# Teachable-AI-Lab/RAG-Cobweb

Measured on AMD Instinct MI355X. Metric: queries/sec + recall@10 vs FAISS-flat, 1M×768 corpus, 1/2/4/8 MI355X, higher is better.
Workload: dtype f32

## Files before the change

### rag-cobweb_amd/csrc/cwq_mfma.hip

```cpp
#include <hip/hip_runtime.h>
#include <math.h>
#include <stdint.h>

#include <algorithm>
#include <type_traits>

#include "cwq_internal.h"

namespace cwq {

typedef __bf16 bf16x8 __attribute__((ext_vector_type(8)));
typedef float f32x16 __attribute__((ext_vector_type(16)));
typedef float f32x4 __attribute__((ext_vector_type(4)));
typedef int i32x4 __attribute__((ext_vector_type(4)));
typedef float f32x2 __attribute__((ext_vector_type(2)));
typedef __attribute__((address_space(3))) void lds_void;
typedef __attribute__((address_space(1))) void glb_void;

#define CWQ_INF __builtin_inff()

__device__ __forceinline__ float up(double v) { return (float)(v * (1.0 + 0x1p-20)); }

__global__ void rows_prep_kernel(const float* __restrict__ mean, int D, const int64_t* __restrict__ nodes, int64_t n,
                                 const float* __restrict__ c, int DP, int DPB, int64_t ld, float* Mf, __bf16* Mb,
// ... 246 lines not shown
    float sc;
    i8_split_wave([&](int d) { return (valid && d < a.D) ? xq[d] - cq[d] : 0.f; }, a.DPB,
                  reinterpret_cast<int8_t*>(a.Xq) + r * a.DPB, sv, shi, slo, sc);
    if (lane == 0) a.qinfo8[r] = make_float4((float)sv, up(sqrt(shi)), up(sqrt(slo)), sc);
  }
  if (!valid) return;
  if (tid < 5) a.qcnt[(size_t)tid * a.nq + r] = 0;
  if (r == 0 && tid == 5) a.qcnt[(size_t)5 * a.nq] = 0;
  if (a.NI == 0) return;
  float* part = s_sb + 2 * DQ;
  for (int t = tid; t < a.NI * NV16; t += 256) {
    const int n = t / NV16, v = t - n * NV16;
    float pp;
#pragma unroll
    for (int j = 0; j < 16; ++j) {
      const int d = v * 16 + j;
      const float x = xq[d];
      const float tt = fmaf(x, a.A[(size_t)d * a.ld + n], -a.B[(size_t)d * a.ld + n]);
      pp = (j == 0) ? tt * tt : fmaf(tt, tt, pp);
    }
    part[t] = pp;
  }
  __syncthreads();
  float* Pl = part + a.NI * NV16;
  for (int lv = 0; lv < a.nlev; ++lv) {
    for (int i = a.lv0[lv] + tid; i < a.lv0[lv + 1]; i += 256) {
      const float acc = sum_in_order(part + i * NV16, NV16);
      const float lp = -0.5f * (a.logdet_int[i] + acc);
      const int p = a.par_int[i];
      const float P = p >= 0 ? fmaf(a.w_int[i], lp, Pl[p]) : a.w_int[i] * lp;
      Pl[i] = P;
      a.P[(size_t)r * a.ldP + i] = P;
    }
    __syncthreads();
  }
}

hipError_t launch_sb_prep(const SbPrepArgs& a, hipStream_t s) {
  const size_t lds = ((size_t)2 * std::max(a.DP, a.DPB) + (size_t)a.NI * (a.DP / 16) + a.NI) * 4;
  if (a.nq <= 0 || a.nq_pad < a.nq16 || a.nq16 < a.nq || a.DP % 16 || a.NI > kSbMaxNI || a.nlev > kSbMaxNI ||
      lds > 65536)
    return hipErrorInvalidValue;
  hipLaunchKernelGGL(sb_prep_kernel, dim3((unsigned)a.nq_pad), dim3(256), lds, s, a);
  return hipGetLastError();
}

__device__ __forceinline__ void prefix_step(float pl, float ph, float w, float& lo, float& hi) {
  const float a = w >= 0.f ? lo : hi, b = w >= 0.f ? hi : lo;
  const float m = 0x1p-21f * (fmaxf(fabsf(pl), fabsf(ph)) + fabsf(w) * fmaxf(fabsf(lo), fabsf(hi)));
  lo = fmaf(w, a, pl) - m;
  hi = fmaf(w, b, ph) + m;
}

__global__ void int_prep_kernel(const float* __restrict__ mean, const VarSrc var, int D,
                                const int64_t* __restrict__ nodes, int64_t n, const float* __restrict__ c,
                                const float* __restrict__ logdet, const int* __restrict__ par_int,
                                const float* __restrict__ w_int, int DP, int DPB2, int64_t ld, __bf16* Mb2, RowF* rf,
                                float* Ar, float* Br, float gamma) {
  const int lane = threadIdx.x & 63;
  const int64_t r = blockIdx.x * (int64_t)kWavesPerWG + (threadIdx.x >> 6);
  if (r >= ld) return;
  double shi = 0.0, slo = 0.0, cn = 0.0, mn = 0.0;
  float wmax = 0.f;
  for (int k = lane; k < DPB2; k += kWave) {
    const int d = k < DP ? k : k - DP;
    const bool ok = r < n && k < 2 * DP && d < D;
    float v = 0.f;
    if (ok) {
      const int64_t o = nodes[r] * (int64_t)D + d;
      const float A = 1.0f / sqrtf(var.at(nodes[r], d, D));
      const float w = A * A;
      const float mu = mean[o];
      const float mc = mu - c[d];
      if (k < DP) {
        v = -0.5f * w;
        const double am = fabs((double)mu) + fabs((double)c[d]);
        cn += (double)mc * (double)mc * (double)w;
        mn += (double)w * am * am;
        wmax = fmaxf(wmax, w);
        Ar[r * DP + d] = A;
        Br[r * DP + d] = mu * A;
      } else {
        v = mc * w;
      }
    } else if (r < n && k < DP) {
      Ar[r * DP + k] = 0.f;
      Br[r * DP + k] = 0.f;
    }
    const __bf16 h = (__bf16)v;
    const float hf = (float)h;
    const float lo = v - hf;
    if (Mb2) Mb2[r * DPB2 + k] = h;
    shi += (double)hf * (double)hf;
    slo += (double)lo * (double)lo;
  }
  for (int off = 32; off > 0; off >>= 1) {
    shi += __shfl_xor(shi, off, 64);
    slo += __shfl_xor(slo, off, 64);
    cn += __shfl_xor(cn, off, 64);
    mn += __shfl_xor(mn, off, 64);
    wmax = fmaxf(wmax, __shfl_xor(wmax, off, 64));
  }
  if (lane == 0) {
    RowF f;
    if (r < n) {
      const double bh = sqrt(shi) * (1.0 + 0x1p-20), bl = sqrt(slo) * (1.0 + 0x1p-20);
      f.R0 = up(mn);
      f.beta = up(bl + (double)gamma * bh);
      f.delta = up(bh + bl);
      f.rn2 = (float)cn;
      f.hs = wmax;
      f.hl = logdet[r];
      f.invL = w_int[r];
      f.par = par_int[r];
    } else {
      f = RowF{0.f, 0.f, 0.f, 0.f, 0.f, 0.f, 0.f, -2};
    }
    if (rf) rf[r] = f;
  }
}

hipError_t launch_int_prep(const float* mean, const VarSrc& var, int D, const int64_t* nodes, int64_t n,
                           const float* c, const float* logdet, const int* par_int, const float* w_int, int DP, int DPB2,
                           int64_t ld, void* Mb2, RowF* rf, float* Ar, float* Br, float gamma, hipStream_t s) {
  if (ld <= 0) return hipSuccess;
  hipLaunchKernelGGL(int_prep_kernel, dim3((unsigned)((ld + 3) / 4)), dim3(256), 0, s, mean, var, D, nodes, n, c,
                     logdet, par_int, w_int, DP, DPB2, ld, (__bf16*)Mb2, rf, Ar, Br, gamma);
  return hipGetLastError();
}

__global__ void int_path_prep_kernel(const float* __restrict__ mean, const VarSrc var, int D,
                                     const int64_t* __restrict__ nodes, const int* __restrict__ rows, int64_t n,
                                     const float* __restrict__ c, const float* __restrict__ logdet,
                                     const int* __restrict__ par_int, const float* __restrict__ w_int, int DP, int DPB2,
                                     int64_t ld, __bf16* Mb2, RowF* rf, float gamma) {
  const int lane = threadIdx.x & 63;
  const int64_t r = blockIdx.x * (int64_t)kWavesPerWG + (threadIdx.x >> 6);
  if (r >= ld) return;
  const int i = r < n ? rows[r] : -1;
  double K0 = 0.0, Z0 = 0.0, Z3 = 0.0;
  int depth = 0;
  for (int a = i; a >= 0 && par_int[a] >= 0; a = par_int[a]) {
    ++depth;
    const int64_t nd = nodes[a];
    double cn = 0.0, mn = 0.0;
    float wmax = 0.f;
    for (int d = lane; d < D; d += kWave) {
      const float A = 1.0f / sqrtf(var.at(nd, d, D));
      const float w = A * A;
      const float mu = mean[nd * (int64_t)D + d];
      const float mc = mu - c[d];
      const double am = fabs((double)mu) + fabs((double)c[d]);
      cn += (double)mc * (double)mc * (double)w;
      mn += (double)w * am * am;
      wmax = fmaxf(wmax, w);
    }
    for (int off = 32; off > 0; off >>= 1) {
      cn += __shfl_xor(cn, off, 64);
      mn += __shfl_xor(mn, off, 64);
      wmax = fmaxf(wmax, __shfl_xor(wmax, off, 64));
    }
    const double wa = (double)w_int[a], ld_a = (double)logdet[a];
    K0 += -0.5 * wa * (ld_a + cn);
    Z0 += fabs(wa) * (mn + fabs(ld_a) + cn);
    Z3 += fabs(wa) * (double)wmax;
  }
  double shi = 0.0, slo = 0.0;
  for (int k = lane; k < DPB2; k += kWave) {
    const int d = k < DP ? k : k - DP;
    double acc = 0.0;
    if (k < 2 * DP && d < D)
      for (int a = i; a >= 0 && par_int[a] >= 0; a = par_int[a]) {
        const int64_t nd = nodes[a];
        const float A = 1.0f / sqrtf(var.at(nd, d, D));
        const float w = A * A;
        const float v = k < DP ? -0.5f * w : (mean[nd * (int64_t)D + d] - c[d]) * w;
        acc += (double)w_int[a] * (double)v;
      }
    const float v = (float)acc;
    const __bf16 h = (__bf16)v;
    const float hf = (float)h;
    const float lo = v - hf;
    Mb2[r * DPB2 + k] = h;
    shi += (double)hf * (double)hf;
    slo += (double)lo * (double)lo;
  }
  for (int off = 32; off > 0; off >>= 1) {
    shi += __shfl_xor(shi, off, 64);
    slo += __shfl_xor(slo, off, 64);
  }
  if (lane == 0) {
    RowF f = RowF{0.f, 0.f, 0.f, 0.f, 0.f, 0.f, 0.f, -2};
    if (i >= 0) {
      f.par = par_int[i];
      if (f.par >= 0) {
        const double bh = sqrt(shi) * (1.0 + 0x1p-20), bl = sqrt(slo) * (1.0 + 0x1p-20);
        const double cz = 1.02 * (0x1p-12 + depth * 0x1p-24);
        f.beta = up(bl + (double)gamma * bh);
        f.delta = up(bh + bl);
        f.rn2 = (float)K0;
        f.hs = up(cz * Z3);
        f.R0 = up(cz * Z0 + 0x1p-23 * fabs(K0));
        f.hl = up(depth * 0x1p-24 + 0x1p-22);
      }
    }
    rf[r] = f;
  }
}

hipError_t launch_int_path_prep(const float* mean, const VarSrc& var, int D, const int64_t* nodes, const int* rows,
                                int64_t n, const float* c, const float* logdet, const int* par_int,
                                const float* w_int, int DP, int DPB2, int64_t ld, void* Mb2, RowF* rf, float gamma,
                                hipStream_t s) {
  if (ld <= 0) return hipSuccess;
  hipLaunchKernelGGL(int_path_prep_kernel, dim3((unsigned)((ld + 3) / 4)), dim3(256), 0, s, mean, var, D, nodes, rows,
                     n, c, logdet, par_int, w_int, DP, DPB2, ld, (__bf16*)Mb2, rf, gamma);
  return hipGetLastError();
}

__global__ void query_prep2_kernel(const float* __restrict__ q, int64_t nq, int D, const float* __restrict__ c,
                                   int DP, int DPB2, int64_t nq_pad, __bf16* Xb2, float4* qinfo) {
  const int lane = threadIdx.x & 63;
  const int64_t r = blockIdx.x * (int64_t)kWavesPerWG + (threadIdx.x >> 6);
  if (r >= nq_pad) return;
  double shi = 0.0, slo = 0.0, sx = 0.0;
  for (int k = lane; k < DPB2; k += kWave) {
    const int d = k < DP ? k : k - DP;
    float v = 0.f;
    if (r < nq && k < 2 * DP && d < D) {
      const float x = q[r * D + d];
      const float xc = x - c[d];
      v = k < DP ? xc * xc : xc;
      if (k < DP) sx += (double)x * (double)x + (double)xc * (double)xc;
    }
    const __bf16 h = (__bf16)v;
    const float hf = (float)h;
    const float lo = v - hf;
    Xb2[r * DPB2 + k] = h;
    shi += (double)hf * (double)hf;
    slo += (double)lo * (double)lo;
  }
  for (int off = 32; off > 0; off >>= 1) {
    shi += __shfl_xor(shi, off, 64);
    slo += __shfl_xor(slo, off, 64);
    sx += __shfl_xor(sx, off, 64);
  }
  if (lane == 0) qinfo[r] = make_float4(up(sx), up(sqrt(shi)), up(sqrt(slo)), 0.f);
}

hipError_t launch_query_prep2(const float* q, int64_t nq, int D, const float* c, int DP, int DPB2, int64_t nq_pad,
                              void* Xb2, float4* qinfo, hipStream_t s) {
  hipLaunchKernelGGL(query_prep2_kernel, dim3((unsigned)((nq_pad + 3) / 4)), dim3(256), 0, s, q, nq, D, c, DP, DPB2,
                     nq_pad, (__bf16*)Xb2, qinfo);
  return hipGetLastError();
}

__global__ void prefix_bounds_kernel(float* Plo, float* Phi, int64_t ldP, int nq, int i0, int i1,
                                     const int* __restrict__ par_int, const float* __restrict__ w_int,
                                     const float* __restrict__ logdet_int, const float* __restrict__ Sroot) {
  const int n = i1 - i0;
  const int64_t total = (int64_t)n * nq;
  for (int64_t t = blockIdx.x * (int64_t)blockDim.x + threadIdx.x; t < total; t += (int64_t)gridDim.x * blockDim.x) {
    const int q = (int)(t / n);
    const int i = i0 + (int)(t % n);
    const size_t o = (size_t)q * ldP + i;
    const int p = par_int[i];
    const float w = w_int[i];
    if (p < 0) {
      const float lp = -0.5f * (logdet_int[i] + Sroot[q]);
      const float P = w * lp;
      Plo[o] = P;
      Phi[o] = P;
      continue;
    }
    const size_t op = (size_t)q * ldP + p;
    float lo = Plo[o], hi = Phi[o];
    prefix_step(Plo[op], Phi[op], w, lo, hi);
    Plo[o] = lo;
    Phi[o] = hi;
  }
}

hipError_t launch_prefix_bounds(float* Plo, float* Phi, int64_t ldP, int nq, int i0, int i1, const int* par_int,
                                const float* w_int, const float* logdet_int, const float* Sroot, hipStream_t s) {
  const int64_t total = (int64_t)(i1 - i0) * nq;
  if (total <= 0) return hipSuccess;
  dim3 grid((unsigned)std::min<int64_t>((total + 255) / 256, 8192));
  hipLaunchKernelGGL(prefix_bounds_kernel, grid, dim3(256), 0, s, Plo, Phi, ldP, nq, i0, i1, par_int, w_int,
                     logdet_int, Sroot);
  return hipGetLastError();
}

constexpr int FT = kFgTile;
constexpr int FK = 32;
constexpr int FNBUF = 4;
constexpr int FSTAGE = 2 * FT * FK * 2;
constexpr int OFF_QV = FNBUF * FSTAGE;
constexpr int OFF_QI = OFF_QV + FT * 4;
constexpr int OFF_PI = OFF_QI + FT * 16;
constexpr int OFF_PL = OFF_PI + FT * 4;
constexpr int OFF_REC = OFF_PL + FT * 4;
constexpr int OFF_CNT = OFF_REC + kFgCap * 16;
constexpr int FLDS = OFF_CNT + 128;


__device__ __forceinline__ void int_bounds(float dot, float4 qi, const RowF& f, float gamma, float& lo, float& hi) {
  (void)gamma;
  const float S0 = fmaf(-2.f, dot, f.rn2);
  const float E = 2.f * (fmaf(qi.y, f.beta, qi.z * f.delta) + 0x1p-23f * fabsf(dot)) + 0x1p-20f * fabsf(f.rn2) +
                  0x1p-12f * fmaf(f.hs, qi.x, f.R0);
  const float Eu = E * (1.f + 0x1p-20f);
  const float Shi = (S0 + Eu) * (1.f + 0x1p-22f);
  const float Slo = fmaxf(0.f, (S0 - Eu) * (1.f - 0x1p-22f));
  const float m = 0x1p-20f * (fabsf(f.hl) + Shi);
  hi = -0.5f * (f.hl + Slo) + m;
  lo = -0.5f * (f.hl + Shi) - m;
}

__device__ __forceinline__ void fg_decode(const FgArgs& a, int xcd, int i, int& qt, int& rt) {
  const int qg = xcd % a.qgroups, rg = xcd / a.qgroups;
  const int nqt_g = (a.n_qt + a.qgroups - 1) / a.qgroups;
  const int nrt_g = (a.n_rt + a.rgroups - 1) / a.rgroups;
  const int q_lo = qg * nqt_g, r_lo = rg * nrt_g;
  const int nq_l = max(1, min(nqt_g, a.n_qt - q_lo));
  const int nr_l = max(1, min(nrt_g, a.n_rt - r_lo));
  if (a.order == 1) {
    qt = q_lo + i / nr_l;
    rt = a.rt_off + r_lo + i % nr_l;
  } else {
    qt = q_lo + i % nq_l;
    rt = a.rt_off + r_lo + i / nq_l;
  }
}

__device__ __forceinline__ int fg_count(const FgArgs& a, int xcd) {
  const int qg = xcd % a.qgroups, rg = xcd / a.qgroups;
  const int nqt_g = (a.n_qt + a.qgroups - 1) / a.qgroups;
  const int nrt_g = (a.n_rt + a.rgroups - 1) / a.rgroups;
  const int nq_l = max(0, min(nqt_g, a.n_qt - qg * nqt_g));
  const int nr_l = max(0, min(nrt_g, a.n_rt - rg * nrt_g));
  return nq_l * nr_l;
}

#ifndef FG_STAMP
#define FG_STAMP 0
#endif
#ifndef FG_LEAN
#define FG_LEAN 1
#endif
#define FG_CSLOT (FG_LEAN && !RAW && MODE == 0 && (tile_no & 1) ? 9 : 0)
__device__ __forceinline__ int fg_swz(int r) { return (4 - ((r >> 2) & 3)) & 3; }

template <int ES = 2>
__device__ __forceinline__ void fg_stage(const __bf16* __restrict__ Xb, const __bf16* __restrict__ Mb, int DPB, int q0,
                                         int r0, int k0, char* sb, int wave, const uint32_t* loff, int ipart = -1) {
  const char* gA = reinterpret_cast<const char*>(Xb) + ((size_t)q0 * DPB + k0) * ES;
  const char* gB = reinterpret_cast<const char*>(Mb) + ((size_t)r0 * DPB + k0) * ES;
#pragma unroll
  for (int i = 0; i < 2; ++i) {
    if (ipart >= 0 && i != ipart) continue;
    __builtin_amdgcn_global_load_lds((glb_void*)(gA + loff[i]), (lds_void*)(sb + (wave * 32 + i * 16) * 64), 16, 0, 0);
    __builtin_amdgcn_global_load_lds((glb_void*)(gB + loff[i]), (lds_void*)(sb + FT * 64 + (wave * 32 + i * 16) * 64), 16,
                                     0, 0);
  }
}

__device__ __forceinline__ TileF fg_tile_const(const TileF* p, int i) {
  static_assert(sizeof(TileF) == 32, "TileF is 8 dwords");
  typedef const __attribute__((address_space(4))) int* cip;
  const cip src = (cip)(uintptr_t)(p + i);
  TileF t;
  int* d = reinterpret_cast<int*>(&t);
#pragma unroll
  for (int k = 0; k < 8; ++k) d[k] = src[k];
  return t;
}

template <bool I8 = false>
__device__ __forceinline__ bool fg_raw_bounds(const FgArgs& a, int q, int row, float d, float ex, float& u,
                                              float& lo) {
  const RowF f = (I8 ? a.rf8 : a.rf)[row];
  if (f.par < -1) return false;
  const TileF tf = a.tf[row / kFgTile];
  float Pq = 0.f, Pql = 0.f;
  if (tf.par >= 0) {
    if (a.pb.dot) {
      pathb_bounds(a.pb, q, tf.par, Pql, Pq);
    } else {
      Pq = (a.Phi ? a.Phi : a.P)[pidx(a.ldP, a.pT, q, tf.par)];
      Pql = a.P[pidx(a.ldP, a.pT, q, tf.par)];
    }
  }
  const float pi = __fmul_rn(Pq, tf.invL), pl = __fmul_rn(Pql, tf.invL);
  fg_bounds2(d, ex, (I8 ? a.qinfo8 : a.qinfo)[q], f, pi, pl, a.eps_n, a.slack, u, lo);
  return u >= a.T[(size_t)q * a.ldT];
}

template <int MODE, bool ALLUNI, bool RAW = false, bool I8 = false>
__global__ __launch_bounds__(512) void fgemm_kernel(const __bf16* __restrict__ Xb, const __bf16* __restrict__ Mb,
                                                    const FgArgs a) {
  static_assert(!I8 || RAW, "int8 operands: raw-record launches only");
  typedef typename std::conditional<I8, i32x4, bf16x8>::type frag_t;
  typedef typename std::conditional<I8, i32x4, f32x4>::type acc_t;
  constexpr int ES = I8 ? 1 : 2;
  constexpr int SK = 64 / ES;
  __shared__ __attribute__((aligned(16))) char smem[FLDS + (I8 ? 2 * FT * 8 : 0)];
  const int tid = threadIdx.x;
  const int lane = tid & 63;
  const int wave = __builtin_amdgcn_readfirstlane(tid >> 6);
  const int wq = wave & 1, wr = wave >> 1;
  const int xcd = blockIdx.x & 7;
  const int lw = blockIdx.x >> 3;
  const int nw_x = ((int)gridDim.x - xcd + 7) >> 3;
  const int ntl = fg_count(a, xcd);
  const bool dyn = a.order == 2;
  if (!dyn && lw >= ntl) return;
  const int nk = a.DPB / SK;
  float* s_qv = reinterpret_cast<float*>(smem + OFF_QV);
  float4* s_qi = reinterpret_cast<float4*>(smem + OFF_QI);
  float* s_pi = reinterpret_cast<float*>(smem + OFF_PI);
  float* s_pl = reinterpret_cast<float*>(smem + OFF_PL);
  const float* Pu = a.Phi ? a.Phi : a.P;
  auto pboth = [&](int64_t q, int p, float& lo, float& hi) {
    if (a.pb.dot) {
      pathb_bounds(a.pb, q, p, lo, hi);
    } else {
      lo = a.P[pidx(a.ldP, a.pT, q, p)];
      hi = Pu[pidx(a.ldP, a.pT, q, p)];
    }
  };
  int4* s_rec = reinterpret_cast<int4*>(smem + OFF_REC);
  int* s_cnt = reinterpret_cast<int*>(smem + OFF_CNT);
  static_assert(!RAW || (MODE == 0 && ALLUNI), "raw records: all-uniform filter launches only");
  static_assert(kFgCap == 512, "the record flush copies one record per thread");
  auto flush_records = [&](int cnt) {
    const int n = min(cnt, kFgCap);
    if (tid == 0) {
      int chunk = s_cnt[1], fill = s_cnt[2];
      int n1 = chunk >= 0 ? min(n, kFgChunk - fill) : 0;
      int base1 = chunk * kFgChunk + fill, base2 = 0, nw = n;
      fill += n1;
      if (n > n1) {
        if (chunk >= 0) a.chunk_fill[chunk] = fill;
        const int c2 = atomicAdd(a.gctr, 1);
        if ((int64_t)(c2 + 1) * kFgChunk > a.rec_cap) {
          chunk = -1;
          fill = 0;
          nw = n1;
        } else {
          chunk = c2;
          fill = n - n1;
          base2 = c2 * kFgChunk;
        }
      }
      s_cnt[1] = chunk;
      s_cnt[2] = fill;
      s_cnt[3] = base1;
      s_cnt[4] = n1;
      s_cnt[5] = nw;
      s_cnt[6] = base2;
    }
    __syncthreads();
    const int nw = s_cnt[5], n1 = s_cnt[4];
    if (tid < nw) a.rec[tid < n1 ? s_cnt[3] + tid : s_cnt[6] + (tid - n1)] = s_rec[tid];
    else if (tid < n) a.qover[s_rec[tid].x] = 1;
    if (tid == 0) s_cnt[0] = 0;
  };
  uint32_t loff[2];
#pragma unroll
  for (int i = 0; i < 2; ++i) {
    const int row = wave * 32 + i * 16 + (lane >> 2);
    loff[i] = (uint32_t)((row * a.DPB + (((lane & 3) ^ fg_swz(row)) * (16 / ES))) * ES);
  }
  const int r16 = lane & 15, c16 = lane >> 4;
  const int foff16 = r16 * 64 + ((c16 ^ fg_swz(r16)) << 4);

  int i = lw;
  if (dyn) {
    if (tid == 0) s_cnt[8] = atomicAdd(&a.tctr[xcd], 1);
    __syncthreads();
    i = __builtin_amdgcn_readfirstlane(s_cnt[8]);
    if (i >= ntl) return;
  }
  int next_i = dyn ? ntl : i + nw_x;
  int ic_i = i, ic_k = 0, ic_qt, ic_rt, issued = 0, gs = 0;
  fg_decode(a, xcd, ic_i, ic_qt, ic_rt);
  auto issue_next = [&]() {
    if (ic_i == -2) {
      ic_i = next_i;
      if (ic_i < ntl) fg_decode(a, xcd, ic_i, ic_qt, ic_rt);
    }
    if (ic_i >= ntl) return;
    if (!(a.dbg & 1)) fg_stage<ES>(Xb, Mb, a.DPB, ic_qt * FT, ic_rt * FT, ic_k * SK, smem + (issued & (FNBUF - 1)) * FSTAGE, wave, loff);
    ++issued;
    if (++ic_k == nk) {
      ic_k = 0;
      ic_i = -2;
    }
  };
  issue_next();
  issue_next();
  if (!I8 || nk >= 3) issue_next();
  int qt, rt;
  int tile_no = 0;
  (void)tile_no;
  fg_decode(a, xcd, i, qt, rt);
  if (tid == 0) {
    s_cnt[0] = 0;
    s_cnt[9] = 0;
    s_cnt[1] = -1;
    s_cnt[2] = 0;
  }
  if (RAW && lane == 0) s_cnt[16 + wave] = 0;
  acc_t acc[8][4];
#if FG_STAMP
  unsigned long long* tsp = (a.stamp && blockIdx.x < 64 && tid == 0) ? a.stamp + 16384 + (size_t)blockIdx.x * 128 : nullptr;
#define FG_TS(k)                                                                  \
  do {                                                                            \
    if (tsp && tile_no < 16) tsp[tile_no * 8 + (k)] = __builtin_amdgcn_s_memtime(); \
  } while (0)
#else
#define FG_TS(k) \
  do {           \
  } while (0)
#endif
  for (;;) {
    FG_TS(0);
    const int q0 = qt * FT, r0 = rt * FT;
    TileF tf;
    if (MODE == 0) tf = fg_tile_const(I8 ? a.tf8 : a.tf, rt);
    else tf.uniform = 0;
    const bool uni = ALLUNI || tf.uniform != 0;
    const bool multi = !ALLUNI && tf.uniform == 2;
    int claimv = 0;
    if (dyn && tid == 0) {
      int z;
      asm volatile("v_mov_b32 %0, 0" : "=v"(z));
      claimv = atomicAdd(a.tctr + xcd + z, 1);
    }
    const int qs = q0 + tid;
    float4 qi = make_float4(0.f, 0.f, 0.f, 0.f);
    float Tq = CWQ_INF, Pq = 0.f, Pql = 0.f;
    float2 rw8 = make_float2(-CWQ_INF, 0.f);
    (void)rw8;
    if (tid < FT) {
      qi = (I8 ? a.qinfo8 : a.qinfo)[qs];
      if (qs < a.nq && MODE == 0) Tq = a.T[(size_t)qs * a.ldT];
      if (uni && tf.par >= 0 && qs < a.nq) {
        if (a.pb.dot) {
          pathb_bounds(a.pb, qs, tf.par, Pql, Pq);
        } else {
          Pq = Pu[pidx(a.ldP, a.pT, qs, tf.par)];
          Pql = a.P[pidx(a.ldP, a.pT, qs, tf.par)];
        }
      }
      if (I8 && r0 + tid < a.nrows) rw8 = make_float2(a.rf[r0 + tid].R0, a.rf8[r0 + tid].R0);
    }
    float R0[4], SR[4];
    (void)SR;
#pragma unroll
    for (int jb = 0; jb < 4; ++jb) {
      if (I8) break;
      const int r = r0 + wr * 64 + jb * 16 + r16;
      R0[jb] = (uni && r < a.nrows) ? a.rf[r].R0 : RAW ? -CWQ_INF : 0.f;
    }
    float* const s_qvt = RAW && (tile_no & 1) ? reinterpret_cast<float*>(smem + OFF_QI) : s_qv;
    if (tid < FT) {
      const float T = Tq;
      if constexpr (I8) {
        (tile_no & 1 ? s_pl : s_pi)[tid] = qi.w;
        reinterpret_cast<float2*>(smem + FLDS)[(tile_no & 1) * FT + tid] = rw8;
      }
      qi.w = T;
      if (!RAW) s_qi[tid] = qi;
      auto qv_of = [&](float pi) {
        const float tpg = (T - pi) / tf.g;
        float v = qi.x * (0.5f - 0.5f * a.eps_n) - 1.5f * a.slack * qi.x + tpg - a.slack * fabsf(pi) / tf.g -
                  qi.y * tf.beta_max - qi.z * tf.delta_max;
        v -= 4.f * a.gamma * (fabsf(v) + qi.x + fabsf(tpg) + fabsf(pi) / tf.g);
        return v == v ? v : CWQ_INF;
      };
      float pi = 0.f, qv = CWQ_INF;
      if (uni) {
        pi = Pq * tf.invL;
        if (qs < a.nq && T > -CWQ_INF) {
          qv = qv_of(pi);
          if (multi) {
            const float2 pm = a.pmm[(size_t)rt * a.ldq + qs];
            const float A = qi.x * (0.5f - 0.5f * a.eps_n) - 1.5f * a.slack * qi.x - qi.y * tf.beta_max -
                            qi.z * tf.delta_max;
            const float M = fmaxf(fabsf(pm.x), fabsf(pm.y));
            const float v1L = A + (T - pm.y) / tf.g - a.slack * M / tf.g;
            const float v1U = A + (T - pm.x) / tf.g;
            const float tpm = fmaxf(fabsf(T - pm.x), fabsf(T - pm.y)) / tf.g;
            const float v = v1L - 4.f * a.gamma * (fmaxf(fabsf(v1L), fabsf(v1U)) + qi.x + tpm + M / tf.g);
            qv = v == v ? fminf(qv, v) : CWQ_INF;
          }
        }
      }
      if (!RAW) {
        s_pi[tid] = pi;
        s_pl[tid] = uni ? Pql * tf.invL : 0.f;
      }
      if (MODE == 2) s_pl[tid] = qs < a.nq ? a.root_w * (-0.5f * (a.root_ld + a.Sroot[qs])) : 0.f;
      s_qvt[tid] = qv;
    }
    if (dyn && tid == 0) s_cnt[8] = claimv;
    __syncthreads();
    FG_TS(1);
    if (dyn) next_i = __builtin_amdgcn_readfirstlane(s_cnt[8]);
    if (FG_LEAN && !RAW && MODE == 0 && tid == 0 && tile_no > 0) s_cnt[(tile_no & 1) ? 0 : 9] = 0;
    if (RAW) {
      const int cnt = s_cnt[0];
      if (cnt >= kFgCap / 2) flush_records(cnt);
    }
#pragma unroll
    for (int ib = 0; ib < 8; ++ib) {
      if constexpr (I8) {
#pragma unroll
        for (int jb = 0; jb < 4; ++jb) acc[ib][jb] = acc_t{0, 0, 0, 0};
      } else {
        const float4 qv4 = uni ? *reinterpret_cast<const float4*>(s_qvt + wq * 128 + ib * 16 + 4 * c16)
                               : make_float4(0.f, 0.f, 0.f, 0.f);
#pragma unroll
        for (int jb = 0; jb < 4; ++jb) {
          acc[ib][jb][0] = R0[jb] - qv4.x;
          acc[ib][jb][1] = R0[jb] - qv4.y;
          acc[ib][jb][2] = R0[jb] - qv4.z;
          acc[ib][jb][3] = R0[jb] - qv4.w;
        }
      }
    }
    frag_t xa1[8], xb0[4];
    const int grp = wave >> 2;
    auto sbar = [&]() {
      __builtin_amdgcn_sched_barrier(0);
      __builtin_amdgcn_s_barrier();
      __builtin_amdgcn_sched_barrier(0);
    };
    if (grp) sbar();
#if FG_STAMP
    const bool stp = a.stamp && blockIdx.x < 16 && (wave & 3) == 0 && lane == 0 && tile_no >= 4 && tile_no < 6;
    unsigned long long* sp =
        stp ? a.stamp + ((((size_t)blockIdx.x * 2 + (tile_no - 4)) * 2 + (wave >> 2)) * 32) * 6 : nullptr;
#define FG_ST(k)                                                               \
  do {                                                                         \
    if (stp && t < 32) sp[t * 6 + (k)] = __builtin_amdgcn_s_memtime();         \
  } while (0)
#else
#define FG_ST(k) \
  do {           \
  } while (0)
#endif
    for (int t = 0; t < nk; ++t) {
      FG_ST(0);
      const char* sb = smem + (gs & (FNBUF - 1)) * FSTAGE;
      issue_next();
      if (!(a.dbg & 128)) {
        const char* sA = sb + wq * 128 * 64 + foff16;
        const char* sB = sb + FT * 64 + wr * 64 * 64 + foff16;
#pragma unroll
        for (int ib = 0; ib < 8; ++ib) xa1[ib] = *reinterpret_cast<const frag_t*>(sA + ib * 1024);
#pragma unroll
        for (int jb = 0; jb < 4; ++jb) xb0[jb] = *reinterpret_cast<const frag_t*>(sB + jb * 1024);
      }
      ++gs;
      const int n_out = issued - gs - 1;
      if (a.dbg & 256) asm volatile("s_waitcnt lgkmcnt(0)" ::: "memory");
      else if (n_out >= 2) asm volatile("s_waitcnt vmcnt(8) lgkmcnt(0)" ::: "memory");
      else if (n_out == 1) asm volatile("s_waitcnt vmcnt(4) lgkmcnt(0)" ::: "memory");
      else asm volatile("s_waitcnt vmcnt(0) lgkmcnt(0)" ::: "memory");
      FG_ST(1);
      sbar();
      FG_ST(2);
#pragma unroll
      for (int ib = 0; ib < 8; ++ib)
#pragma unroll
        for (int jb = 0; jb < 4; ++jb) {
          if constexpr (I8) acc[ib][jb] = __builtin_amdgcn_mfma_i32_16x16x64_i8(xa1[ib], xb0[jb], acc[ib][jb], 0, 0, 0);
          else acc[ib][jb] = __builtin_amdgcn_mfma_f32_16x16x32_bf16(xa1[ib], xb0[jb], acc[ib][jb], 0, 0, 0);
        }
      FG_ST(3);
      if (t + 1 < nk || grp == 0) sbar();
      FG_ST(4);
    }
#undef FG_ST
    FG_TS(2);
    float* wsc = reinterpret_cast<float*>(smem + ((gs - 1) & (FNBUF - 1)) * FSTAGE) + wave * 1024;
    bool anyb[4][2];
    if (a.dbg & 2) goto flush;
    if (MODE == 2 && a.pT) {
      int par[4], rid[4];
#pragma unroll
      for (int jb = 0; jb < 4; ++jb) {
        const int r = r0 + wr * 64 + jb * 16 + r16;
        par[jb] = r < a.nrows ? a.rf[r].par : -2;
        rid[jb] = r < a.nrows ? a.row_id[r] : -1;
      }
#pragma unroll
      for (int ib = 0; ib < 8; ++ib) {
        const int ql = wq * 128 + ib * 16 + 4 * c16;
        const int q = q0 + ql;
        if (q >= a.ldlb) continue;
#pragma unroll
        for (int jb = 0; jb < 4; ++jb) {
          if (par[jb] < -1 || rid[jb] < 0) continue;
          const size_t o = (size_t)rid[jb] * a.ldlb + q;
          const float4 v = par[jb] < 0 ? *reinterpret_cast<const float4*>(s_pl + ql)
                                       : make_float4(acc[ib][jb][0], acc[ib][jb][1], acc[ib][jb][2], acc[ib][jb][3]);
          *reinterpret_cast<float4*>(a.lb + o) = v;
        }
      }
      goto flush;
    }
    if (MODE == 2) {
      const int rl = r0 + wr * 64 + lane;
      const RowF f = rl < a.nrows ? a.rf[rl] : RowF{0.f, 0.f, 0.f, 0.f, 0.f, 0.f, 0.f, -2};
      const int rid = a.row_id ? (rl < a.nrows ? a.row_id[rl] : -1) : rl;
#pragma unroll
      for (int ib = 0; ib < 8; ++ib) {
#pragma unroll
        for (int jb = 0; jb < 4; ++jb)
#pragma unroll
          for (int j = 0; j < 4; ++j) wsc[(4 * c16 + j) * 64 + jb * 16 + r16] = acc[ib][jb][j];
        __builtin_amdgcn_fence(__ATOMIC_RELEASE, "wavefront");
        __builtin_amdgcn_wave_barrier();
        __builtin_amdgcn_fence(__ATOMIC_ACQUIRE, "wavefront");
#pragma unroll 4
        for (int e = 0; e < 16; ++e) {
          const int ql = wq * 128 + ib * 16 + e;
          const int q = q0 + ql;
          if (f.par >= -1 && q < a.nq) {
            const float d0 = wsc[e * 64 + lane];
            float lo, hi;
            if (f.par < 0) {
              lo = hi = s_pl[ql];
            } else if (a.path_sum) {
              path_bounds(d0, s_qi[ql], f, s_pl[ql], lo, hi);
            } else {
              int_bounds(d0, s_qi[ql], f, a.gamma, lo, hi);
              if (f.par == 0) prefix_step(s_pl[ql], s_pl[ql], f.invL, lo, hi);
            }
            a.lb[(size_t)q * a.ldlb + rid] = lo;
            a.lb_hi[(size_t)q * a.ldlb + rid] = hi;
          }
        }
        __builtin_amdgcn_wave_barrier();
      }
      goto flush;
    }
    if (MODE == 1 && a.lbg == 4 && !a.pb.dot) {
      int rrow[4];
      float pa[4], pb[4];
#pragma unroll
      for (int jb = 0; jb < 4; ++jb) {
        const int r = r0 + wr * 64 + jb * 16 + r16;
        const int rr = a.rowmap ? a.rowmap[r] : (r < a.nrows ? r : -1);
        const RowF f = rr >= 0 ? a.rf[rr] : RowF{-CWQ_INF, 0.f, 0.f, 0.f, 0.f, 0.f, 0.f, -2};
        rrow[jb] = f.par >= -1 ? rr : -1;
        pa[jb] = fmaf(f.hs, f.rn2, f.hl);
        pb[jb] = -2.f * f.hs;
      }
      const int g = (r0 + wr * 64) / 4 + r16;
#pragma unroll
      for (int ib = 0; ib < 8; ++ib)
#pragma unroll
        for (int j = 0; j < 4; ++j) {
          const int ql = wq * 128 + ib * 16 + 4 * c16 + j;
          const int q = q0 + ql;
          int best = -1;
          float bk = -CWQ_INF;
#pragma unroll
          for (int jb = 0; jb < 4; ++jb) {
            const float pk = fmaf(pb[jb], acc[ib][jb][j], pa[jb]);
            if (rrow[jb] >= 0 && (best < 0 || pk > bk)) {
              bk = pk;
              best = jb;
            }
          }
          float m = -CWQ_INF;
          if (best >= 0) {
            int rb = rrow[0];
            float d0 = acc[ib][0][j];
#pragma unroll
            for (int jb = 1; jb < 4; ++jb)
              if (best == jb) {
                rb = rrow[jb];
                d0 = acc[ib][jb][j];
              }
            const RowF fb = a.rf[rb];
            const float4 qi = s_qi[ql];
            float pi = 0.f;
            if (fb.par >= 0 && q < a.nq) pi = a.P[pidx(a.ldP, a.pT, q, fb.par)] * fb.invL;
            float u;
            fg_bounds(d0, 0x1p-23f * fabsf(d0), qi, fb, pi, a.eps_n, a.slack, u, m);
            if (a.cat && fb.par >= 0 && q < a.nq) m = fminf(m, (a.BFt ? a.BFt : a.P)[pidx(a.ldP, a.pT, q, fb.par)]);
          }
          a.lb[(size_t)q * a.ldlb + g] = m;
        }
      goto flush;
    }
    if (MODE == 0 && uni) {
      bool any = false;
      const float* const s_sx = (tile_no & 1) ? s_pl : s_pi;
      auto pre8 = [](float t, float sx, float R, float qv) { return fmaf(t, sx, R) - qv; };
      uint32_t sbm = 0;
      if constexpr (RAW) {
#pragma clang fp contract(off)
        if constexpr (I8) {
#pragma unroll
          for (int jb = 0; jb < 4; ++jb) {
            const float2 rw = reinterpret_cast<const float2*>(smem + FLDS)[(tile_no & 1) * FT + wr * 64 + jb * 16 + r16];
            R0[jb] = rw.x;
            SR[jb] = rw.y;
          }
#pragma unroll
          for (int ib = 0; ib < 8; ++ib)
#pragma unroll
            for (int jb = 0; jb < 4; ++jb) {
              const f32x2 sr2 = {SR[jb], SR[jb]};
#pragma unroll
              for (int h = 0; h < 4; h += 2) {
                const f32x2 t = f32x2{(float)acc[ib][jb][h], (float)acc[ib][jb][h + 1]} * sr2;
                acc[ib][jb][h] = __float_as_int(t.x);
                acc[ib][jb][h + 1] = __float_as_int(t.y);
              }
            }
        }
#pragma unroll
        for (int ib = 0; ib < 8; ++ib) {
          const int ql = wq * 128 + ib * 16 + 4 * c16;
          f32x2 qv2[2] = {}, sx2[2] = {};
          if constexpr (I8) {
            const float4 qv4 = *reinterpret_cast<const float4*>(s_qvt + ql);
            const float4 sx4 = *reinterpret_cast<const float4*>(s_sx + ql);
            qv2[0] = f32x2{qv4.x, qv4.y};
            qv2[1] = f32x2{qv4.z, qv4.w};
            sx2[0] = f32x2{sx4.x, sx4.y};
            sx2[1] = f32x2{sx4.z, sx4.w};
          }
#pragma unroll
          for (int jb = 0; jb < 4; ++jb) {
            f32x2 p[2];
#pragma unroll
            for (int h = 0; h < 2; ++h) {
              if constexpr (I8) {
                const f32x2 t = {__int_as_float(acc[ib][jb][2 * h]), __int_as_float(acc[ib][jb][2 * h + 1])};
                p[h] = __builtin_elementwise_fma(t, sx2[h], f32x2{R0[jb], R0[jb]}) - qv2[h];
              } else {
                p[h] = f32x2{(float)acc[ib][jb][2 * h], (float)acc[ib][jb][2 * h + 1]};
              }
            }
            const f32x2 m2 = __builtin_elementwise_max(p[0], p[1]);
            if (__ballot(__builtin_fmaxf(m2.x, m2.y) >= 0.f) != 0) sbm |= 1u << (jb * 8 + ib);
          }
        }
        any = sbm != 0;
      } else {
#pragma unroll
        for (int jb = 0; jb < 4; ++jb)
#pragma unroll
          for (int hf = 0; hf < 2; ++hf) {
            float m = -CWQ_INF;
#pragma unroll
            for (int ib = hf * 4; ib < hf * 4 + 4; ++ib)
              m = __builtin_fmaxf(m, __builtin_fmaxf(__builtin_fmaxf(acc[ib][jb][0], acc[ib][jb][1]),
                                                     __builtin_fmaxf(acc[ib][jb][2], acc[ib][jb][3])));
            anyb[jb][hf] = __ballot(m >= 0.f) != 0;
            any = any || anyb[jb][hf];
          }
      }
      FG_TS(3);
      if (!any) goto flush;
      if (RAW) {
        int4* const wrec = reinterpret_cast<int4*>(wsc);
        uint32_t todo = sbm;
#pragma unroll 1
        while (todo) {
          const int sb = __builtin_ctz(todo);
          todo &= todo - 1;
          const int jb = sb >> 3, ib = sb & 7;
          float d0j[4] = {0.f, 0.f, 0.f, 0.f}, Rv = 0.f;
#define FG_SB(JB, IB)                                                                                   \
  case (JB) * 8 + (IB):                                                                                 \
    _Pragma("unroll") for (int j = 0; j < 4; ++j)                                                       \
        d0j[j] = I8 ? __int_as_float(acc[IB][JB][j]) : (float)acc[IB][JB][j];                           \
    Rv = R0[JB];                                                                                        \
    break;
#define FG_SB8(JB) FG_SB(JB, 0) FG_SB(JB, 1) FG_SB(JB, 2) FG_SB(JB, 3) FG_SB(JB, 4) FG_SB(JB, 5) FG_SB(JB, 6) FG_SB(JB, 7)
          switch (sb) {
            FG_SB8(0) FG_SB8(1) FG_SB8(2) FG_SB8(3)
          }
#undef FG_SB8
#undef FG_SB
          const int r = r0 + wr * 64 + jb * 16 + r16;
          const int ql = wq * 128 + ib * 16 + 4 * c16;
          const float4 qv4 = *reinterpret_cast<const float4*>(s_qvt + ql);
          const float qvj[4] = {qv4.x, qv4.y, qv4.z, qv4.w};
          float4 sx4 = make_float4(0.f, 0.f, 0.f, 0.f);
          if (I8) sx4 = *reinterpret_cast<const float4*>(s_sx + ql);
          const float sxj[4] = {sx4.x, sx4.y, sx4.z, sx4.w};
          bool ovf = false;
#pragma unroll
          for (int j = 0; j < 4; ++j)
            if (I8 ? pre8(d0j[j], sxj[j], Rv, qvj[j]) >= 0.f : d0j[j] >= 0.f) {
              const float d0 = d0j[j];
              float d, ex;
              if (I8) {
                d = __fmul_rn(d0, sxj[j]);
                ex = 0x1p-21f * fabsf(d);
              } else {
                const float init = Rv - qvj[j];
                d = d0 - init;
                ex = a.gamma * fabsf(init) + 0x1p-23f * (fabsf(d0) + fabsf(init));
              }
              const int4 rv = make_int4(q0 + ql + j, r, __float_as_int(d), __float_as_int(ex));
              const int slot = atomicAdd(&s_cnt[0], 1);
              if (slot < kFgCap) {
                s_rec[slot] = rv;
              } else {
                wrec[atomicAdd(&s_cnt[16 + wave], 1)] = rv;
                ovf = true;
              }
            }
          if (__builtin_expect(__any(ovf), 0)) {
            __builtin_amdgcn_fence(__ATOMIC_RELEASE, "wavefront");
            __builtin_amdgcn_wave_barrier();
            __builtin_amdgcn_fence(__ATOMIC_ACQUIRE, "wavefront");
            const int no = s_cnt[16 + wave];
#pragma unroll 1
            for (int k = lane; k < no; k += 64) {
              const int4 rv = wrec[k];
              float u, lo;
              if (fg_raw_bounds<I8>(a, rv.x, rv.y, __int_as_float(rv.z), __int_as_float(rv.w), u, lo)) {
                const int gs = atomicAdd(&a.gctr[1], 1);
                if (gs < a.dir_cap) a.rec_dir[gs] = rv;
                else a.qover[rv.x] = 1;
              }
            }
            __builtin_amdgcn_wave_barrier();
            if (lane == 0) s_cnt[16 + wave] = 0;
            __builtin_amdgcn_fence(__ATOMIC_RELEASE, "wavefront");
          }
        }
        goto flush;
      }
    } else {
#pragma unroll
      for (int jb = 0; jb < 4; ++jb) anyb[jb][0] = anyb[jb][1] = true;
    }
#pragma unroll
    for (int jb = 0; jb < 4; ++jb) {
      if (!anyb[jb][0] && !anyb[jb][1]) continue;
      const int r = r0 + wr * 64 + jb * 16 + r16;
      const int rr = a.rowmap ? a.rowmap[r] : (r < a.nrows ? r : -1);
      const RowF f = rr >= 0 ? a.rf[rr] : RowF{-CWQ_INF, 0.f, 0.f, 0.f, 0.f, 0.f, 0.f, -2};
      const bool usable = f.par >= -1;
      const RowF fpar = (MODE == 0 && a.pb.dot && f.par > 0) ? a.pb.nrf[f.par]
                                                           : RowF{0.f, 0.f, 0.f, 0.f, 0.f, 0.f, 0.f, -1};
      auto pboth_row = [&](int64_t q, float& lo, float& hi) {
        if (a.pb.dot) pathb_bounds_f(a.pb, q, f.par, fpar, lo, hi);
        else pboth(q, f.par, lo, hi);
      };
#pragma unroll
      for (int hf = 0; hf < 2; ++hf) {
        if (!anyb[jb][hf]) continue;
#pragma unroll
        for (int k = 0; k < 4; ++k)
#pragma unroll
          for (int j = 0; j < 4; ++j) wsc[(k * 4 + j) * 64 + lane] = acc[hf * 4 + k][jb][j];
#pragma unroll 1
        for (int e = 0; e < 16; ++e) {
          const float d0 = wsc[e * 64 + lane];
          const int ql = wq * 128 + (hf * 4 + (e >> 2)) * 16 + 4 * c16 + (e & 3);
          const int q = q0 + ql;
            if (MODE == 2) {
              if (usable && q < a.nq && r < a.nrows) {
                float lo, hi;
                if (f.par < 0) {
                  lo = hi = s_pl[ql];
                } else {
                  int_bounds(d0, s_qi[ql], f, a.gamma, lo, hi);
                  if (f.par == 0) prefix_step(s_pl[ql], s_pl[ql], f.invL, lo, hi);
                }
                a.lb[(size_t)q * a.ldlb + r] = lo;
                a.lb_hi[(size_t)q * a.ldlb + r] = hi;
              }
            } else if (MODE == 1) {
              float lo = -CWQ_INF;
              if (usable) {
                const float4 qi = s_qi[ql];
                float pi = 0.f;
                if (f.par >= 0 && q < a.nq) {
                  float plo_, phi_;
                  pboth(q, f.par, plo_, phi_);
                  pi = plo_ * f.invL;
                }
                float u;
                fg_bounds(d0, 0x1p-23f * fabsf(d0), qi, f, pi, a.eps_n, a.slack, u, lo);
                if (a.cat && f.par >= 0 && q < a.nq) lo = fminf(lo, (a.BFt ? a.BFt : a.P)[pidx(a.ldP, a.pT, q, f.par)]);
              }
              a.lb[(size_t)q * a.ldlb + r] = lo;
            } else if (usable && q < a.nq && (!uni || d0 >= 0.f)) {
              const float4 qi = s_qi[ql];
              float d, ex, pi, pl;
              if (uni) {
                const float init = f.R0 - s_qv[ql];
                d = d0 - init;
                ex = a.gamma * fabsf(init) + 0x1p-23f * (fabsf(d0) + fabsf(init));
                if (!ALLUNI && multi) {
                  float plo_, phi_;
                  pboth_row(q, plo_, phi_);
                  pi = phi_ * f.invL;
                  pl = plo_ * f.invL;
                } else {
                  pi = s_pi[ql];
                  pl = s_pl[ql];
                }
              } else {
                d = d0;
                ex = 0x1p-23f * fabsf(d0);
                float plo_ = 0.f, phi_ = 0.f;
                if (f.par >= 0) pboth_row(q, plo_, phi_);
                pi = phi_ * f.invL;
                pl = plo_ * f.invL;
              }
              float u, lo;
              fg_bounds2(d, ex, qi, f, pi, pl, a.eps_n, a.slack, u, lo);
              if (a.cat && f.par >= 0) {
                const float bp = (a.BFt ? a.BFt : a.P)[pidx(a.ldP, a.pT, q, f.par)];
                u = fminf(u, bp);
                lo = fminf(lo, bp);
              }
              if (u >= qi.w) {
                const int4 rv = make_int4(q, r, __float_as_int(u), __float_as_int(lo));
                const int slot = atomicAdd(&s_cnt[FG_CSLOT], 1);
                if (slot < kFgCap) {
                  s_rec[slot] = rv;
                } else {
                  const int gs = atomicAdd(&a.gctr[1], 1);
                  if (gs < a.dir_cap) a.rec_dir[gs] = rv;
                  else a.qover[q] = 1;
                }
              }
            }
          }
        }
    }
  flush:
    FG_TS(4);
    if (MODE == 0 && !RAW) {
      __syncthreads();
      FG_TS(5);
      const int cnt = s_cnt[FG_CSLOT];
      const int n = min(cnt, kFgCap);
      if (FG_LEAN && n == 0) goto next_tile;
      if (tid == 0) {
        int chunk = s_cnt[1], fill = s_cnt[2];
        int n1 = chunk >= 0 ? min(n, kFgChunk - fill) : 0;
        int base1 = chunk * kFgChunk + fill, base2 = 0, lost = 0;
        fill += n1;
        if (n > n1) {
          if (chunk >= 0) a.chunk_fill[chunk] = fill;
          const int c2 = atomicAdd(a.gctr, 1);
          if ((int64_t)(c2 + 1) * kFgChunk > a.rec_cap) {
            lost = 1;
            chunk = -1;
            fill = 0;
            s_cnt[5] = n1;
          } else {
            chunk = c2;
            fill = n - n1;
            base2 = c2 * kFgChunk;
            s_cnt[5] = n;
          }
        } else {
          s_cnt[5] = n;
        }
        s_cnt[1] = chunk;
        s_cnt[2] = fill;
        s_cnt[3] = base1;
        s_cnt[4] = n1;
        s_cnt[6] = base2;
        s_cnt[7] = lost;
      }
      __syncthreads();
      const int nw = s_cnt[5], n1 = s_cnt[4];
      if (tid < nw) a.rec[tid < n1 ? s_cnt[3] + tid : s_cnt[6] + (tid - n1)] = s_rec[tid];
      if (s_cnt[7] && tid < FT && q0 + tid < a.nq) a.qover[q0 + tid] = 1;
    }
  next_tile:
    i = next_i;
    FG_TS(6);
    ++tile_no;
    if (i >= ntl) break;
    if (!dyn) next_i = i + nw_x;
    fg_decode(a, xcd, i, qt, rt);
    if (!RAW && (MODE != 0 || !FG_LEAN)) {
      __syncthreads();
      if (tid == 0) s_cnt[0] = 0;
    }
  }
  if (RAW) {
    __syncthreads();
    const int cnt = s_cnt[0];
    if (cnt > 0) flush_records(cnt);
  }
  if (MODE == 0 && tid == 0 && s_cnt[1] >= 0) a.chunk_fill[s_cnt[1]] = s_cnt[2];
}

int fgemm_dpb(int D) {
  const int g = 2 * FK;
  const int r = (D + g - 1) / g * g;
  const int lo = 4 * FK;
  return r > lo ? r : lo;
}

hipError_t launch_fgemm(const void* Xb, const void* Mb, const FgArgs& a, int n_wg, hipStream_t s) {
  if (a.DPB != fgemm_dpb(a.DPB) || a.n_qt <= 0 || a.n_rt <= 0) return hipErrorInvalidValue;
  if (a.qgroups * a.rgroups != 8) return hipErrorInvalidValue;
  n_wg = std::max(8, n_wg / 8 * 8);
  if (a.mode == 1)
    hipLaunchKernelGGL((fgemm_kernel<1, false>), dim3((unsigned)n_wg), dim3(512), 0, s, (const __bf16*)Xb,
                       (const __bf16*)Mb, a);
  else if (a.mode == 2)
    hipLaunchKernelGGL((fgemm_kernel<2, false>), dim3((unsigned)n_wg), dim3(512), 0, s, (const __bf16*)Xb,
                       (const __bf16*)Mb, a);
  else if ((a.raw && !a.all_uniform) || (a.i8 && (!a.raw || a.DPB % 64 || !a.qinfo8 || !a.rf8 || !a.tf8)))
    return hipErrorInvalidValue;
  else if (a.i8)
    hipLaunchKernelGGL((fgemm_kernel<0, true, true, true>), dim3((unsigned)n_wg), dim3(512), 0, s, (const __bf16*)Xb,
                       (const __bf16*)Mb, a);
  else if (a.raw)
    hipLaunchKernelGGL((fgemm_kernel<0, true, true>), dim3((unsigned)n_wg), dim3(512), 0, s, (const __bf16*)Xb,
                       (const __bf16*)Mb, a);
  else if (a.all_uniform)
    hipLaunchKernelGGL((fgemm_kernel<0, true>), dim3((unsigned)n_wg), dim3(512), 0, s, (const __bf16*)Xb,
                       (const __bf16*)Mb, a);
  else
    hipLaunchKernelGGL((fgemm_kernel<0, false>), dim3((unsigned)n_wg), dim3(512), 0, s, (const __bf16*)Xb,
                       (const __bf16*)Mb, a);
  return hipGetLastError();
}

__device__ __forceinline__ void bucket_one(const int4 r, int capq, int* qcnt, int* qover, int* crow, float* cu,
                                           float* cl) {
  const int q = r.x;
  const int slot = atomicAdd(&qcnt[q], 1);
  if (slot < capq) {
    const size_t o = (size_t)q * capq + slot;
    crow[o] = r.y;
    cu[o] = __int_as_float(r.z);
    cl[o] = __int_as_float(r.w);
  } else {
    qover[q] = 1;
  }
}

__global__ __launch_bounds__(256) void bucket_kernel(const int4* __restrict__ rec, const int* __restrict__ gctr,
                                                     const int* __restrict__ chunk_fill, int64_t rec_cap,
                                                     const int4* __restrict__ rec_dir, int dir_cap, int capq,
                                                     int* qcnt, int* qover, int* crow, float* cu, float* cl) {
  const int64_t stride = (int64_t)gridDim.x * blockDim.x;
  const int64_t g0 = blockIdx.x * (int64_t)blockDim.x + threadIdx.x;
  const int64_t n_rec = min((int64_t)gctr[0] * kFgChunk, rec_cap);
  for (int64_t g = g0; g < n_rec; g += stride)
    if ((int)(g % kFgChunk) < chunk_fill[g / kFgChunk]) bucket_one(rec[g], capq, qcnt, qover, crow, cu, cl);
  const int n_dir = min(gctr[1], dir_cap);
  for (int64_t d = g0; d < n_dir; d += stride) bucket_one(rec_dir[d], capq, qcnt, qover, crow, cu, cl);
}

__device__ __forceinline__ void bucket_raw_one(const FgArgs& a, const int4 r, int capq, int* qcnt, int* crow,
                                               float* cu, float* cl) {
  const int q = r.x, row = r.y;
  if ((unsigned)q >= (unsigned)a.nq || (unsigned)row >= (unsigned)a.nrows) return;
  float u, lo;
  const float d = __int_as_float(r.z), ex = __int_as_float(r.w);
  if (a.i8 ? fg_raw_bounds<true>(a, q, row, d, ex, u, lo) : fg_raw_bounds<false>(a, q, row, d, ex, u, lo))
    bucket_one(make_int4(q, row, __float_as_int(u), __float_as_int(lo)), capq, qcnt, a.qover, crow, cu, cl);
}

__global__ __launch_bounds__(256) void bucket_raw_kernel(const FgArgs a, int capq, int* qcnt, int* crow, float* cu,
                                                         float* cl) {
  const int64_t stride = (int64_t)gridDim.x * blockDim.x;
  const int64_t g0 = blockIdx.x * (int64_t)blockDim.x + threadIdx.x;
  const int64_t n_rec = min((int64_t)a.gctr[0] * kFgChunk, a.rec_cap);
  for (int64_t g = g0; g < n_rec; g += stride)
    if ((int)(g % kFgChunk) < a.chunk_fill[g / kFgChunk]) bucket_raw_one(a, a.rec[g], capq, qcnt, crow, cu, cl);
  const int n_dir = min(a.gctr[1], a.dir_cap);
  for (int64_t d = g0; d < n_dir; d += stride) bucket_raw_one(a, a.rec_dir[d], capq, qcnt, crow, cu, cl);
}

hipError_t launch_bucket_raw(const FgArgs& a, int capq, int* qcnt, int* crow, float* cu, float* cl, hipStream_t s) {
  const int64_t n = a.rec_cap + a.dir_cap;
  const unsigned grid = (unsigned)std::min<int64_t>((n + 255) / 256, 2048);
  hipLaunchKernelGGL(bucket_raw_kernel, dim3(grid), dim3(256), 0, s, a, capq, qcnt, crow, cu, cl);
  return hipGetLastError();
}

hipError_t launch_bucket(const int4* rec, const int* gctr, const int* chunk_fill, int64_t rec_cap, const int4* rec_dir,
                         int dir_cap, int capq, int* qcnt, int* qover, int* crow, float* cu, float* cl, hipStream_t s) {
  const int64_t n = rec_cap + dir_cap;
  const unsigned grid = (unsigned)std::min<int64_t>((n + 255) / 256, 2048);
  hipLaunchKernelGGL(bucket_kernel, dim3(grid), dim3(256), 0, s, rec, gctr, chunk_fill, rec_cap, rec_dir, dir_cap,
                     capq, qcnt, qover, crow, cu, cl);
  return hipGetLastError();
}

__global__ __launch_bounds__(256) void select_kernel(const float* __restrict__ u, int64_t ldu, int nq, int nrows,
                                                     int Kp, float* cu, int* crow) {
  const int lane = threadIdx.x & 63;
  const int q = blockIdx.x * kWavesPerWG + __builtin_amdgcn_readfirstlane((int)(threadIdx.x >> 6));
  if (q >= nq) return;
  float lk;
  int lr;
  select_wave(u + (size_t)q * ldu, nrows, Kp, lane, lk, lr);
  cu[(size_t)q * 64 + lane] = lk;
  crow[(size_t)q * 64 + lane] = lr;
}

hipError_t launch_select(const float* u, int64_t ldu, int nq, int nrows, int Kp, float* cu, int* crow, hipStream_t s) {
  hipLaunchKernelGGL(select_kernel, dim3((unsigned)((nq + kWavesPerWG - 1) / kWavesPerWG)), dim3(256), 0, s, u, ldu,
                     nq, nrows, Kp, cu, crow);
  return hipGetLastError();
}

constexpr int kPrQ = 32, kPrTiles = 4, kPrSpan = 128;
__global__ __launch_bounds__(256) void tile_prange_kernel(const float* __restrict__ P, const float* __restrict__ Phi,
                                                          int64_t ldP, int nq, const TileF* __restrict__ tf, int n_rt,
                                                          float2* __restrict__ pmm, int64_t ldq) {
  __shared__ float s_lo[kPrQ][kPrSpan + 1], s_hi[kPrQ][kPrSpan + 1];
  const int tid = threadIdx.x;
  const int runs = (n_rt + kPrTiles - 1) / kPrTiles;
  const int q0 = (blockIdx.x / runs) * kPrQ;
  const int t0 = (blockIdx.x % runs) * kPrTiles, t1 = min(t0 + kPrTiles, n_rt);
  int pa = 0x7fffffff, pb = -1;
  for (int t = t0; t < t1; ++t) {
    const TileF T = tf[t];
    if (T.uniform == 2) {
      pa = min(pa, T.par);
      pb = max(pb, T.par_hi);
    }
// ... 1004 lines not shown
```

Measured before the change: 1.055 million.

## Emit int8 raw-mode candidates inline via ballot-compacted wave staging

In the int8 raw path, surviving candidates of a flagged 16x16 sub-block are now written immediately during the ballot scan into a per-wave staging buffer, with slots computed by mbcnt prefix counts instead of per-lane LDS atomics. At the end the wave reserves space in the shared record list with a single atomic and copies the staged records over, spilling any excess through the bounds check. Sub-blocks that do not fit the staging area fall back to the old switch-based second pass. The goal is to remove the per-candidate shared-memory atomics and the re-extraction pass from the accumulator registers, at the cost of extra register pressure and code size inside the unrolled scan loop.

New measurement: 1.090 million, median of 6. 1.03x the previous value.

```diff
diff --git a/rag-cobweb_amd/csrc/cwq_mfma.hip b/rag-cobweb_amd/csrc/cwq_mfma.hip
--- a/rag-cobweb_amd/csrc/cwq_mfma.hip
+++ b/rag-cobweb_amd/csrc/cwq_mfma.hip
@@ -572,6 +572,8 @@
 constexpr int OFF_REC = OFF_PL + FT * 4;
 constexpr int OFF_CNT = OFF_REC + kFgCap * 16;
 constexpr int FLDS = OFF_CNT + 128;
+constexpr int kFgStage = FSTAGE / 8 / 16;
+static_assert(kFgStage == 256, "a full 16 x 16 sub-block (4 values x 64 lanes) fits the staging area");
 
 
 __device__ __forceinline__ void int_bounds(float dot, float4 qi, const RowF& f, float gamma, float& lo, float& hi) {
@@ -1074,7 +1076,20 @@
       bool any = false;
       const float* const s_sx = (tile_no & 1) ? s_pl : s_pi;
       auto pre8 = [](float t, float sx, float R, float qv) { return fmaf(t, sx, R) - qv; };
-      uint32_t sbm = 0;
+      uint32_t todo = 0;
+      int n_w = 0;
+      int4* const wrec = reinterpret_cast<int4*>(wsc);
+      auto raw_de = [&](float d0, float Rv, float qv, float sx, float& d, float& ex) {
+        if (I8) {
+          d = __fmul_rn(d0, sx);
+          ex = 0x1p-21f * fabsf(d);
+        } else {
+          const float init = Rv - qv;
+          d = d0 - init;
+          ex = a.gamma * fabsf(init) + 0x1p-23f * (fabsf(d0) + fabsf(init));
+        }
+      };
+      const int qb = q0 + wq * 128 + 4 * c16, rb = r0 + wr * 64 + r16;
       if constexpr (RAW) {
 #pragma clang fp contract(off)
         if constexpr (I8) {
@@ -1103,9 +1118,9 @@
           f32x2 qv2[2] = {}, sx2[2] = {};
           if constexpr (I8) {
             const float4 qv4 = *reinterpret_cast<const float4*>(s_qvt + ql);
-            const float4 sx4 = *reinterpret_cast<const float4*>(s_sx + ql);
             qv2[0] = f32x2{qv4.x, qv4.y};
             qv2[1] = f32x2{qv4.z, qv4.w};
+            const float4 sx4 = *reinterpret_cast<const float4*>(s_sx + ql);
             sx2[0] = f32x2{sx4.x, sx4.y};
             sx2[1] = f32x2{sx4.z, sx4.w};
           }
@@ -1122,10 +1137,40 @@
               }
             }
             const f32x2 m2 = __builtin_elementwise_max(p[0], p[1]);
-            if (__ballot(__builtin_fmaxf(m2.x, m2.y) >= 0.f) != 0) sbm |= 1u << (jb * 8 + ib);
+            const bool flag = __ballot(__builtin_fmaxf(m2.x, m2.y) >= 0.f) != 0;
+            if constexpr (!I8) {
+              if (flag) todo |= 1u << (jb * 8 + ib);
+              continue;
+            }
+            if (__builtin_expect(flag, 0)) {
+              const float pj[4] = {p[0].x, p[0].y, p[1].x, p[1].y};
+              unsigned long long bj[4];
+              int need = 0;
+#pragma unroll
+              for (int j = 0; j < 4; ++j) {
+                bj[j] = __ballot(pj[j] >= 0.f);
+                need += __builtin_popcountll(bj[j]);
+              }
+              if (n_w + need <= kFgStage) {
+#pragma unroll
+                for (int j = 0; j < 4; ++j) {
+                  if (pj[j] >= 0.f) {
+                    float d, ex;
+                    raw_de(I8 ? __int_as_float(acc[ib][jb][j]) : (float)acc[ib][jb][j], R0[jb], qv2[j >> 1][j & 1],
+                           sx2[j >> 1][j & 1], d, ex);
+                    const int slot = n_w + (int)__builtin_amdgcn_mbcnt_hi((uint32_t)(bj[j] >> 32),
+                                                                         __builtin_amdgcn_mbcnt_lo((uint32_t)bj[j], 0u));
+                    wrec[slot] = make_int4(qb + ib * 16 + j, rb + jb * 16, __float_as_int(d), __float_as_int(ex));
+                  }
+                  n_w += __builtin_popcountll(bj[j]);
+                }
+              } else {
+                todo |= 1u << (jb * 8 + ib);
+              }
+            }
           }
         }
-        any = sbm != 0;
+        any = (n_w | (int)todo) != 0;
       } else {
 #pragma unroll
         for (int jb = 0; jb < 4; ++jb)
@@ -1143,8 +1188,34 @@
       FG_TS(3);
       if (!any) goto flush;
       if (RAW) {
-        int4* const wrec = reinterpret_cast<int4*>(wsc);
-        uint32_t todo = sbm;
+        auto drain = [&](int k0, int k1) {
+#pragma unroll 1
+          for (int k = k0 + lane; k < k1; k += 64) {
+            const int4 rv = wrec[k];
+            float u, lo;
+            if (fg_raw_bounds<I8>(a, rv.x, rv.y, __int_as_float(rv.z), __int_as_float(rv.w), u, lo)) {
+              const int gs = atomicAdd(&a.gctr[1], 1);
+              if (gs < a.dir_cap) a.rec_dir[gs] = rv;
+              else a.qover[rv.x] = 1;
+            }
+          }
+        };
+        if (n_w > 0) {
+          __builtin_amdgcn_fence(__ATOMIC_RELEASE, "wavefront");
+          __builtin_amdgcn_wave_barrier();
+          __builtin_amdgcn_fence(__ATOMIC_ACQUIRE, "wavefront");
+          int base = 0;
+          if (lane == 0) base = atomicAdd(&s_cnt[0], n_w);
+          base = __builtin_amdgcn_readfirstlane(base);
+          const int room = max(0, min(n_w, kFgCap - base));
+#pragma unroll 1
+          for (int k = lane; k < room; k += 64) s_rec[base + k] = wrec[k];
+          if (__builtin_expect(room < n_w, 0)) drain(room, n_w);
+          __builtin_amdgcn_wave_barrier();
+          __builtin_amdgcn_fence(__ATOMIC_RELEASE, "wavefront");
+        }
+        FG_TS(7);
+        if (todo) FG_TS(5);
 #pragma unroll 1
         while (todo) {
           const int sb = __builtin_ctz(todo);
@@ -1174,16 +1245,8 @@
 #pragma unroll
           for (int j = 0; j < 4; ++j)
             if (I8 ? pre8(d0j[j], sxj[j], Rv, qvj[j]) >= 0.f : d0j[j] >= 0.f) {
-              const float d0 = d0j[j];
               float d, ex;
-              if (I8) {
-                d = __fmul_rn(d0, sxj[j]);
-                ex = 0x1p-21f * fabsf(d);
-              } else {
-                const float init = Rv - qvj[j];
-                d = d0 - init;
-                ex = a.gamma * fabsf(init) + 0x1p-23f * (fabsf(d0) + fabsf(init));
-              }
+              raw_de(d0j[j], Rv, qvj[j], sxj[j], d, ex);
               const int4 rv = make_int4(q0 + ql + j, r, __float_as_int(d), __float_as_int(ex));
               const int slot = atomicAdd(&s_cnt[0], 1);
               if (slot < kFgCap) {
@@ -1197,17 +1260,7 @@
             __builtin_amdgcn_fence(__ATOMIC_RELEASE, "wavefront");
             __builtin_amdgcn_wave_barrier();
             __builtin_amdgcn_fence(__ATOMIC_ACQUIRE, "wavefront");
-            const int no = s_cnt[16 + wave];
-#pragma unroll 1
-            for (int k = lane; k < no; k += 64) {
-              const int4 rv = wrec[k];
-              float u, lo;
-              if (fg_raw_bounds<I8>(a, rv.x, rv.y, __int_as_float(rv.z), __int_as_float(rv.w), u, lo)) {
-                const int gs = atomicAdd(&a.gctr[1], 1);
-                if (gs < a.dir_cap) a.rec_dir[gs] = rv;
-                else a.qover[rv.x] = 1;
-              }
-            }
+            drain(0, s_cnt[16 + wave]);
             __builtin_amdgcn_wave_barrier();
             if (lane == 0) s_cnt[16 + wave] = 0;
             __builtin_amdgcn_fence(__ATOMIC_RELEASE, "wavefront");
```
